# NEUROINFORMATICS-GROUP-FAV-KIV-ZCU/EEG_DataAnalysisPackage

Measured on AMD Instinct MI355X. Metric: epochs/sec feature-extracted (whole node) + % HBM roofline, 1/2/4/8 GPUs, higher is better.
Workload: dtype f64

## Files before the change

### eeg_dataanalysispackage_amd/csrc/nn.hip

```cpp
#include <hip/hip_runtime.h>

#include <algorithm>
#include <cstdint>

#include "eegfx.h"
#include "launch.h"

namespace eegfx {

constexpr int kNnThreads = 256;
constexpr int kNnMaxTileRows = 64;
constexpr int kNnMinStagedRows = 8;
constexpr int kNnLdsBytes = 147456;
constexpr int kNnGridCap = 768;
constexpr int kNnAccRegs = 4;
constexpr int kNnPartialDoubles = 8388608;
constexpr int kNnValidateThreads = 256;
constexpr int kNnValidateMaxBlocks = 4096;
constexpr int kNnStatThreads = 256;
constexpr int kNnStatUnroll = 4;
constexpr int kNnStatMaxBlocks = 2048;
constexpr int kNnDirThreads = 1024;

namespace dev {

__device__ __forceinline__ double nn_act(int act, double z) {
  switch (act) {
    case EEGFX_NN_ACT_TANH: return tanh(z);
    case EEGFX_NN_ACT_RELU: return z > 0.0 ? z : (z == z ? 0.0 : z);
    case EEGFX_NN_ACT_IDENTITY: return z;
    case EEGFX_NN_ACT_SOFTPLUS: return (z > 0.0 ? z : 0.0) + log1p(exp(-fabs(z)));
    case EEGFX_NN_ACT_ELU: return z > 0.0 ? z : expm1(z);
    default: return 1.0 / (1.0 + exp(-z));
  }
}

__device__ __forceinline__ double nn_dact(int act, double z, double a) {
  switch (act) {
    case EEGFX_NN_ACT_TANH: return 1.0 - a * a;
    case EEGFX_NN_ACT_RELU: return z > 0.0 ? 1.0 : 0.0;
    case EEGFX_NN_ACT_IDENTITY: return 1.0;
    case EEGFX_NN_ACT_SOFTPLUS: return 1.0 / (1.0 + exp(-z));
    case EEGFX_NN_ACT_ELU: return z > 0.0 ? 1.0 : exp(z);
    default: return a * (1.0 - a);
  }
}

__device__ __forceinline__ double nn_dot(const double* a, const double* w, int ws, int n,
                                         double z) {
  for (int i = 0; i < n; ++i) z = __builtin_fma(a[i], w[(int64_t)i * ws], z);
  return z;
}

__device__ __forceinline__ void nn_stage_weights(const NnNet& net, const NnTile& tl, double* lds,
                                                 const double* __restrict__ params) {
  const int t = threadIdx.x;
  for (int l = 0; l < net.L; ++l) {
    const int no = net.n_out[l], nw = net.n_in[l] * no;
    const double* src = params + net.w_off[l];
    if (l > 0 || tl.w1_lds) {
      int i = t / no, j = t - i * no;
      const int di = kNnThreads / no, dj = kNnThreads - di * no;
      for (int e = t; e < nw; e += kNnThreads) {
        lds[tl.w_lds[l] + i * tl.w_stride[l] + j] = src[e];
        i += di;
        j += dj;
        if (j >= no) {
          j -= no;
          ++i;
        }
      }
    }
    for (int j = t; j < no; j += kNnThreads) lds[tl.b_lds[l] + j] = src[nw + j];
  }
}

__device__ __forceinline__ void nn_load_rows(const NnNet& net, const NnTile& tl, double* lds,
                                             const double* __restrict__ X,
                                             const double* __restrict__ y, int64_t row0,
                                             int rows) {
  const int t = threadIdx.x, d = net.d;
  const double* src = X + row0 * d;
  int r = t / d, c = t - r * d;
  const int dr = kNnThreads / d, dc = kNnThreads - dr * d;
  for (int e = t; e < rows * d; e += kNnThreads) {
    lds[tl.x_off + r * tl.x_stride + c] = src[e];
    r += dr;
    c += dc;
    if (c >= d) {
      c -= d;
      ++r;
    }
  }
  if (y && t < rows) lds[tl.y_off + t] = y[row0 + t];
}

__device__ __forceinline__ void nn_forward(const NnNet& net, const NnTile& tl, double* lds,
                                           const double* __restrict__ params, int rows) {
  const int t = threadIdx.x;
  for (int l = 0; l < net.L; ++l) {
    const int no = net.n_out[l], ni = net.n_in[l], act = net.act[l];
    const int in_off = l == 0 ? tl.x_off : tl.a_off[l - 1];
    const int in_stride = l == 0 ? tl.x_stride : tl.a_stride[l - 1];
    const int os = tl.a_stride[l];
    int r = t / no, j = t - r * no;
    const int dr = kNnThreads / no, dj = kNnThreads - dr * no;
    for (int e = t; e < rows * no; e += kNnThreads) {
      const double* a = lds + in_off + r * in_stride;
      double z = lds[tl.b_lds[l] + j];
      if (l == 0 && !tl.w1_lds)
        z = nn_dot(a, params + net.w_off[0] + j, no, ni, z);
      else
        z = nn_dot(a, lds + tl.w_lds[l] + j, tl.w_stride[l], ni, z);
      lds[tl.z_off[l] + r * os + j] = z;
      if (act != EEGFX_NN_ACT_SOFTMAX) lds[tl.a_off[l] + r * os + j] = nn_act(act, z);
      r += dr;
      j += dj;
      if (j >= no) {
        j -= no;
        ++r;
      }
    }
    __syncthreads();
    if (act == EEGFX_NN_ACT_SOFTMAX) {
      if (t < rows) {
        const double* z = lds + tl.z_off[l] + t * os;
        double* a = lds + tl.a_off[l] + t * os;
        double m = z[0];
        for (int j2 = 1; j2 < no; ++j2) m = fmax(m, z[j2]);
        double s = 0.0;
        for (int j2 = 0; j2 < no; ++j2) {
          const double ez = exp(z[j2] - m);
          a[j2] = ez;
          s += ez;
        }
        for (int j2 = 0; j2 < no; ++j2) a[j2] = a[j2] / s;
      }
      __syncthreads();
    }
  }
}

struct NnTerm {
  int a_off, a_stride, d_off, d_stride;
};
__device__ __forceinline__ NnTerm nn_term(const NnNet& net, const NnTile& tl, int p) {
  int l = 0;
  for (int k = 1; k < net.L; ++k)
    if (p >= net.w_off[k]) l = k;
  const int q = p - net.w_off[l], no = net.n_out[l], nw = net.n_in[l] * no;
  NnTerm tm;
  tm.d_stride = tl.a_stride[l];
  if (q < nw) {
    const int i = q / no;
    tm.d_off = tl.z_off[l] + (q - i * no);
    tm.a_off = (l == 0 ? tl.x_off : tl.a_off[l - 1]) + i;
    tm.a_stride = l == 0 ? tl.x_stride : tl.a_stride[l - 1];
  } else {
    tm.d_off = tl.z_off[l] + (q - nw);
    tm.a_off = -1;
    tm.a_stride = 0;
  }
  return tm;
}
__device__ __forceinline__ double nn_term_sum(const double* lds, const NnTerm& tm, int rows,
                                              double acc) {
  if (tm.a_off >= 0) {
    for (int r = 0; r < rows; ++r)
      acc = __builtin_fma(lds[tm.a_off + r * tm.a_stride], lds[tm.d_off + r * tm.d_stride], acc);
  } else {
    for (int r = 0; r < rows; ++r) acc += lds[tm.d_off + r * tm.d_stride];
  }
  return acc;
}

__device__ __forceinline__ double nn_row_loss(int kind, double p0, double p1, double y0, double y1,
                                              double* g0, double* g1) {
  switch (kind) {
    case EEGFX_NN_LOSS_XENT:
      *g0 = -y0 / p0 + (1.0 - y0) / (1.0 - p0);
      *g1 = -y1 / p1 + (1.0 - y1) / (1.0 - p1);
      return -((y0 * log(p0) + (1.0 - y0) * log(1.0 - p0)) +
               (y1 * log(p1) + (1.0 - y1) * log(1.0 - p1)));
    case EEGFX_NN_LOSS_NLL:
      *g0 = -y0 / p0;
      *g1 = -y1 / p1;
      return -(y0 * log(p0) + y1 * log(p1));
    case EEGFX_NN_LOSS_SQUARED:
      *g0 = 2.0 * (p0 - y0);
      *g1 = 2.0 * (p1 - y1);
      return (p0 - y0) * (p0 - y0) + (p1 - y1) * (p1 - y1);
    default:
      *g0 = p0 - y0;
      *g1 = p1 - y1;
      return ((p0 - y0) * (p0 - y0) + (p1 - y1) * (p1 - y1)) / 2.0;
  }
}

__device__ __forceinline__ void nn_store_loss(const NnTile& tl, double* lds, double my_loss,
                                              double* out) {
  const int t = threadIdx.x;
  __syncthreads();
  if (t < kNnMaxTileRows) lds[tl.loss_off + t] = my_loss;
  __syncthreads();
  if (t == 0) {
    double s = 0.0;
    for (int r = 0; r < kNnMaxTileRows; ++r) s += lds[tl.loss_off + r];
    *out = s;
  }
}

__global__ __launch_bounds__(kNnThreads) void nn_grad_kernel(
    const double* __restrict__ X, const double* __restrict__ y, int64_t n, const NnNet net,
    const NnTile tl, const NnState* __restrict__ st, double* __restrict__ partial) {
  if (st->flag) return;
  extern __shared__ __attribute__((aligned(16))) double nn_lds[];
  double* lds = nn_lds;
  const double* params = (const double*)(st + 1);
  const int t = threadIdx.x, P = net.P, L = net.L;
  double* slab = partial + (int64_t)blockIdx.x * (P + 1);
  nn_stage_weights(net, tl, lds, params);
  NnTerm term[kNnAccRegs];
  double acc[kNnAccRegs];
#pragma unroll
  for (int k = 0; k < kNnAccRegs; ++k) {
    acc[k] = 0.0;
    const int p = t + k * kNnThreads;
    term[k] = nn_term(net, tl, p < P ? p : 0);
  }
  for (int p = t + kNnAccRegs * kNnThreads; p < P; p += kNnThreads) slab[p] = 0.0;
  double my_loss = 0.0;
  const int last = L - 1, out_act = net.act[last];
  for (int64_t row0 = (int64_t)blockIdx.x * tl.rows; row0 < n;
       row0 += (int64_t)gridDim.x * tl.rows) {
    const int rows = (int)(n - row0 < tl.rows ? n - row0 : tl.rows);
    __syncthreads();
    nn_load_rows(net, tl, lds, X, y, row0, rows);
    __syncthreads();
    nn_forward(net, tl, lds, params, rows);
    if (t < rows) {
      const int os = tl.a_stride[last];
      double* z = lds + tl.z_off[last] + t * os;
      const double p0 = lds[tl.a_off[last] + t * os], p1 = lds[tl.a_off[last] + t * os + 1];
      const double y0 = lds[tl.y_off + t], y1 = fabs(1.0 - y0);
      double g0, g1;
      const double loss = nn_row_loss(net.loss, p0, p1, y0, y1, &g0, &g1);
      my_loss += loss;
      double d0, d1;
      if ((net.loss == EEGFX_NN_LOSS_XENT && out_act == EEGFX_NN_ACT_SIGMOID) ||
          (net.loss == EEGFX_NN_LOSS_NLL && out_act == EEGFX_NN_ACT_SOFTMAX)) {
        d0 = p0 - y0;
        d1 = p1 - y1;
      } else if (out_act == EEGFX_NN_ACT_SOFTMAX) {
        const double gp = g0 * p0 + g1 * p1;
        d0 = p0 * (g0 - gp);
        d1 = p1 * (g1 - gp);
      } else {
        d0 = g0 * nn_dact(out_act, z[0], p0);
        d1 = g1 * nn_dact(out_act, z[1], p1);
      }
      z[0] = d0;
      z[1] = d1;
    }
    __syncthreads();
    for (int l = last; l >= 1; --l) {
      const int ni = net.n_in[l], no = net.n_out[l], act = net.act[l - 1];
      const int ps = tl.a_stride[l - 1];
      int r = t / ni, i = t - r * ni;
      const int dr = kNnThreads / ni, di = kNnThreads - dr * ni;
      for (int e = t; e < rows * ni; e += kNnThreads) {
        const double s = nn_dot(lds + tl.z_off[l] + r * tl.a_stride[l],
                                lds + tl.w_lds[l] + i * tl.w_stride[l], 1, no, 0.0);
        double* zp = lds + tl.z_off[l - 1] + r * ps + i;
        *zp = act == EEGFX_NN_ACT_SOFTMAX
                  ? s
                  : s * nn_dact(act, *zp, lds[tl.a_off[l - 1] + r * ps + i]);
        r += dr;
        i += di;
        if (i >= ni) {
          i -= ni;
          ++r;
        }
      }
      __syncthreads();
      if (act == EEGFX_NN_ACT_SOFTMAX) {
        if (t < rows) {
          double* s = lds + tl.z_off[l - 1] + t * ps;
          const double* a = lds + tl.a_off[l - 1] + t * ps;
          double sa = 0.0;
          for (int m = 0; m < ni; ++m) sa = __builtin_fma(s[m], a[m], sa);
          for (int m = 0; m < ni; ++m) s[m] = a[m] * (s[m] - sa);
        }
        __syncthreads();
      }
    }
#pragma unroll
    for (int k = 0; k < kNnAccRegs; ++k)
      if (t + k * kNnThreads < P) acc[k] = nn_term_sum(lds, term[k], rows, acc[k]);
    for (int p = t + kNnAccRegs * kNnThreads; p < P; p += kNnThreads)
      slab[p] = nn_term_sum(lds, nn_term(net, tl, p), rows, slab[p]);
  }
#pragma unroll
  for (int k = 0; k < kNnAccRegs; ++k)
    if (t + k * kNnThreads < P) slab[t + k * kNnThreads] = acc[k];
  nn_store_loss(tl, lds, my_loss, slab + P);
}

__device__ __forceinline__ double nn_updater(int updater, double lr, double mu, int it, double g,
                                             double* s1, double* s2) {
  switch (updater) {
    case EEGFX_NN_UPD_SGD:
      return lr * g;
    case EEGFX_NN_UPD_ADAM: {
      const double b1 = 0.9, b2 = 0.999, t = (double)(it + 1);
      const double m = b1 * *s1 + (1.0 - b1) * g;
      const double v = b2 * *s2 + (1.0 - b2) * (g * g);
      *s1 = m;
      *s2 = v;
      return lr * sqrt(1.0 - pow(b2, t)) / (1.0 - pow(b1, t)) * (m / (sqrt(v) + 1e-8));
    }
    case EEGFX_NN_UPD_ADAGRAD: {
      const double h = *s1 + g * g;
      *s1 = h;
      return lr * g / (sqrt(h) + 1e-6);
    }
    case EEGFX_NN_UPD_RMSPROP: {
      const double r = 0.95 * *s1 + 0.05 * (g * g);
      *s1 = r;
      return lr * g / sqrt(r + 1e-8);
    }
    default: {
      const double v = *s1, vn = mu * v - lr * g;
      *s1 = vn;
      return mu * v - (1.0 + mu) * vn;
    }
  }
}

enum { kVecG = 0, kVecGNew = 1, kVecDir = 2, kVecCand = 3, kVecPOld = 4, kVecGOld = 5,
       kVecS = 6, kVecY = kVecS + kNnLbfgsM };
__device__ __forceinline__ double* nn_opt_vec(const NnOpt* opt, int k, int P) {
  return (double*)(opt + 1) + (int64_t)k * P;
}

__device__ __forceinline__ double nn_partial_mean(const double* __restrict__ partial, int G,
                                                  int64_t n, int P, int p) {
  const int64_t stride = P + 1;
  double s = 0.0;
  for (int b = 0; b < G; ++b) s += partial[b * stride + p];
  return s / (double)n;
}

__device__ __forceinline__ bool nn_last_workgroup(uint32_t* ticket) {
  __syncthreads();
  if (threadIdx.x != 0) return false;
  __threadfence();
  if (atomicAdd(ticket, 1u) != gridDim.x - 1) return false;
  *ticket = 0;
  return true;
}

template <bool OPT>
__global__ __launch_bounds__(kNnThreads) void nn_update_kernel(
    const double* __restrict__ partial, int G, int64_t n, int P, int updater, double lr,
    double mu, NnState* __restrict__ st, NnOpt* __restrict__ opt, double* __restrict__ scores) {
  if (st->flag) return;
  const int it = st->iter;
  const int p = blockIdx.x * kNnThreads + threadIdx.x;
  if (p < P) {
    const double g = nn_partial_mean(partial, G, n, P, p);
    double* w = (double*)(st + 1) + p;
    double* s1 = w + P;
    double* s2 = s1 + P;
    const double u = nn_updater(updater, lr, mu, it, g, s1, s2);
    if constexpr (OPT)
      nn_opt_vec(opt, kVecGNew, P)[p] = u;
    else
      *w = *w - u;
  }
  if (blockIdx.x == 0 && threadIdx.x == 0) {
    if constexpr (OPT)
      opt->score_new = nn_partial_mean(partial, G, n, P, P);
    else if (scores)
      scores[it] = nn_partial_mean(partial, G, n, P, P);
  }
  if (nn_last_workgroup(&st->ticket)) st->iter = it + 1;
}

__device__ __forceinline__ double nn_move(double p, double step, double d) { return p - step * d; }
__device__ __forceinline__ bool nn_finite(double v) { return fabs(v) <= 1.7976931348623157e308; }

__global__ __launch_bounds__(kNnThreads) void nn_score_kernel(
    const double* __restrict__ X, const double* __restrict__ y, int64_t n, const NnNet net,
    const NnTile tl, const NnState* __restrict__ st, const NnOpt* __restrict__ opt,
    double* __restrict__ partial) {
  if (st->flag || opt->line.done) return;
  extern __shared__ __attribute__((aligned(16))) double nn_lds[];
  double* lds = nn_lds;
  const double* params = nn_opt_vec(opt, kVecCand, net.P);
  const int t = threadIdx.x, last = net.L - 1;
  nn_stage_weights(net, tl, lds, params);
  double my_loss = 0.0;
  for (int64_t row0 = (int64_t)blockIdx.x * tl.rows; row0 < n;
       row0 += (int64_t)gridDim.x * tl.rows) {
    const int rows = (int)(n - row0 < tl.rows ? n - row0 : tl.rows);
    __syncthreads();
    nn_load_rows(net, tl, lds, X, y, row0, rows);
    __syncthreads();
    nn_forward(net, tl, lds, params, rows);
    if (t < rows) {
      const int os = tl.a_stride[last];
      const double p0 = lds[tl.a_off[last] + t * os], p1 = lds[tl.a_off[last] + t * os + 1];
      const double y0 = lds[tl.y_off + t], y1 = fabs(1.0 - y0);
      double g0, g1;
      my_loss += nn_row_loss(net.loss, p0, p1, y0, y1, &g0, &g1);
    }
  }
  nn_store_loss(tl, lds, my_loss, partial + (int64_t)blockIdx.x * (net.P + 1) + net.P);
}

__device__ __forceinline__ int nn_line_step(NnLine& ln, double sc, int max_ls, double* move,
                                            NnSearchRec* rec) {
  const double s0 = ln.s0, slope = ln.slope, step = ln.step, prev = ln.sc;
  ln.sc = sc;
  ln.trials += 1;
  rec->trials = ln.trials;
  rec->pad = 0;
  if (sc < ln.best) {
    ln.best = sc;
    ln.best_step = step;
  }
  if (sc <= s0 + 1e-4 * step * slope) {
    ln.done = 1;
    rec->step = *move = step;
    rec->score = sc;
    return 1;
  }
  double tmp;
  if (!nn_finite(sc) || !nn_finite(prev)) {
    tmp = 0.2 * step;
  } else if (step == 1.0) {
    tmp = -slope / (2.0 * (sc - s0 - slope));
  } else {
    const double step2 = ln.step2;
    const double r1 = sc - s0 - step * slope, r2 = ln.sc2 - s0 - step2 * slope;
    const double q1 = r1 / (step * step), q2 = r2 / (step2 * step2);
    const double a = (q1 - q2) / (step - step2);
    const double b = (-step2 * q1 + step * q2) / (step - step2);
    if (a == 0.0) {
      tmp = -slope / (2.0 * b);
    } else {
      const double disc = b * b - 3.0 * a * slope;
      if (disc < 0.0)
        tmp = 0.5 * step;
      else if (b <= 0.0)
        tmp = (-b + sqrt(disc)) / (3.0 * a);
      else
        tmp = -slope / (b + sqrt(disc));
    }
    if (!(tmp < 0.5 * step)) tmp = 0.5 * step;
  }
  ln.step2 = step;
  ln.sc2 = sc;
  ln.step = tmp > 0.1 * step ? tmp : 0.1 * step;
  if (ln.trials < max_ls && !(ln.step < ln.step_min)) {
    *move = ln.step;
    return 0;
  }
  ln.done = 1;
  if (ln.trials == max_ls && ln.best < s0) {
    rec->step = *move = ln.best_step;
    rec->score = ln.best;
    return 1;
  }
  rec->step = *move = 0.0;
  rec->score = s0;
  return 2;
}

__global__ __launch_bounds__(kNnThreads) void nn_search_kernel(
    const double* __restrict__ partial, int G, int64_t n, int P, int max_ls,
    NnState* __restrict__ st, NnOpt* __restrict__ opt, NnSearchRec* __restrict__ search) {
  if (st->flag || opt->line.done) return;
  __shared__ double sh_move;
  __shared__ int sh_mode;
  NnLine ln;
  NnSearchRec rec;
  int it = 0;
  if (threadIdx.x == 0) {
    ln = opt->line;
    it = opt->it;
    double move;
    sh_mode = nn_line_step(ln, nn_partial_mean(partial, G, n, P, P), max_ls, &move, &rec);
    sh_move = move;
  }
  __syncthreads();
  const int mode = sh_mode, k = blockIdx.x * kNnThreads + threadIdx.x;
  if (k < P && mode != 2) {
    double* p = (double*)(st + 1);
    const double v = nn_move(p[k], sh_move, nn_opt_vec(opt, kVecDir, P)[k]);
    if (mode == 1)
      p[k] = v;
    else
      nn_opt_vec(opt, kVecCand, P)[k] = v;
  }
  if (nn_last_workgroup(&opt->ticket)) {
    opt->line = ln;
    if (ln.done) search[it] = rec;
  }
}

template <int N>
__device__ __forceinline__ void nn_block_sum(double (&v)[N], double* red) {
  const int t = threadIdx.x;
#pragma unroll
  for (int k = 0; k < N; ++k) red[k * kNnDirThreads + t] = v[k];
  __syncthreads();
  for (int h = kNnDirThreads / 2; h > 0; h >>= 1) {
    if (t < h) {
#pragma unroll
      for (int k = 0; k < N; ++k) red[k * kNnDirThreads + t] += red[k * kNnDirThreads + t + h];
    }
    __syncthreads();
  }
#pragma unroll
  for (int k = 0; k < N; ++k) v[k] = red[k * kNnDirThreads];
  __syncthreads();
}
__device__ __forceinline__ double nn_block_max(double v, double* red) {
  const int t = threadIdx.x;
  red[t] = v;
  __syncthreads();
  for (int h = kNnDirThreads / 2; h > 0; h >>= 1) {
    if (t < h && (red[t + h] > red[t] || red[t + h] != red[t + h])) red[t] = red[t + h];
    __syncthreads();
  }
  v = red[0];
  __syncthreads();
  return v;
}

__global__ __launch_bounds__(kNnDirThreads) void nn_direction_kernel(
    int P, int algo, int iters, int first, NnState* __restrict__ st, NnOpt* __restrict__ opt,
    double* __restrict__ scores, NnSearchRec* __restrict__ search) {
  if (st->flag) return;
  __shared__ double red[3 * kNnDirThreads];
  constexpr int D = kNnDirThreads, M = kNnLbfgsM;
  const int t = threadIdx.x;
  const double* p = (const double*)(st + 1);
  double* g = nn_opt_vec(opt, kVecG, P);
  const double* gn = nn_opt_vec(opt, kVecGNew, P);
  double* dir = nn_opt_vec(opt, kVecDir, P);
  double* p_old = nn_opt_vec(opt, kVecPOld, P);
  double* g_old = nn_opt_vec(opt, kVecGOld, P);
  const int it = first ? -1 : opt->it;
  const double old = opt->score, score = opt->score_new;
  int hist = opt->hist, head = opt->head;
  double rho_new = 0.0;
  bool stop = false;
  const bool lbfgs = algo == EEGFX_NN_OPT_LBFGS;
  if (first) {
    for (int k = t; k < P; k += D) {
      const double v = gn[k];
      g[k] = v;
      dir[k] = v;
      if (lbfgs) {
        p_old[k] = p[k];
        g_old[k] = v;
      }
    }
  } else {
    if (algo == EEGFX_NN_OPT_CG) {
      double v[2] = {0.0, 0.0};
      for (int k = t; k < P; k += D) {
        v[0] += (gn[k] - g[k]) * gn[k];
        v[1] += g[k] * g[k];
      }
      nn_block_sum(v, red);
      const double q = v[0] / v[1], gamma = q < 0.0 ? 0.0 : q;
      for (int k = t; k < P; k += D) dir[k] = gamma * dir[k] + gn[k];
    } else if (lbfgs) {
      head = hist == 0 ? 0 : (head + 1) % M;
      hist = hist < M ? hist + 1 : M;
      double* s_new = nn_opt_vec(opt, kVecS + head, P);
      double* y_new = nn_opt_vec(opt, kVecY + head, P);
      double v[2] = {0.0, 0.0};
      for (int k = t; k < P; k += D) {
        const double s = p[k] - p_old[k], yv = gn[k] - g_old[k];
        s_new[k] = s;
        y_new[k] = yv;
        v[0] += s * yv;
        v[1] += yv * yv;
        dir[k] = gn[k];
        p_old[k] = p[k];
        g_old[k] = gn[k];
      }
      nn_block_sum(v, red);
      const double sy = v[0] + 1e-5, yy = v[1] + 1e-5;
      rho_new = 1.0 / sy;
      double a[M];
#pragma unroll
      for (int j = 0; j < M; ++j) {
        a[j] = 0.0;
        if (j < hist) {
          const int slot = (head - j + M) % M;
          const double* sv = nn_opt_vec(opt, kVecS + slot, P);
          const double* yv = nn_opt_vec(opt, kVecY + slot, P);
          double d[1] = {0.0};
          for (int k = t; k < P; k += D) d[0] += sv[k] * dir[k];
          nn_block_sum(d, red);
          a[j] = (j == 0 ? rho_new : opt->rho[slot]) * d[0];
          for (int k = t; k < P; k += D) dir[k] -= a[j] * yv[k];
        }
      }
      const double scale = sy / yy;
      for (int k = t; k < P; k += D) dir[k] *= scale;
#pragma unroll
      for (int j = M - 1; j >= 0; --j) {
        if (j < hist) {
          const int slot = (head - j + M) % M;
          const double* sv = nn_opt_vec(opt, kVecS + slot, P);
          const double* yv = nn_opt_vec(opt, kVecY + slot, P);
          double d[1] = {0.0};
          for (int k = t; k < P; k += D) d[0] += yv[k] * dir[k];
          nn_block_sum(d, red);
          const double b = (j == 0 ? rho_new : opt->rho[slot]) * d[0];
          for (int k = t; k < P; k += D) dir[k] += (a[j] - b) * sv[k];
        }
      }
    } else {
      for (int k = t; k < P; k += D) dir[k] = gn[k];
    }
    double asum[1] = {0.0};
    for (int k = t; k < P; k += D) {
      const double v = gn[k];
      g[k] = v;
      asum[0] += fabs(v);
    }
    nn_block_sum(asum, red);
    stop = asum[0] == 0.0;
    if (!(score == 0.0 && old == 0.0) &&
        2.0 * fabs(old - score) <= 1e-5 * (fabs(old) + fabs(score) + 1e-4))
      stop = true;
  }
  const int next = it + 1;
  const bool search_next = !stop && next < iters;
  NnLine ln{};
  if (search_next) {
    double v[2] = {0.0, 0.0};
    double test = 0.0;
    for (int k = t; k < P; k += D) {
      v[0] += dir[k] * dir[k];
      v[1] += dir[k] * g[k];
      const double ap = fabs(p[k]), q = fabs(g[k]) / (ap > 1.0 ? ap : 1.0);
      if (q > test || q != q) test = q;
    }
    nn_block_sum(v, red);
    test = nn_block_max(test, red);
    const double norm = sqrt(v[0]);
    if (norm > 100.0) {
      const double f = 100.0 / norm;
      for (int k = t; k < P; k += D) dir[k] *= f;
    }
    ln.s0 = ln.sc = ln.sc2 = ln.best = score;
    ln.slope = -v[1];
    ln.step_min = 1e-7 / test;
    ln.step = ln.best_step = 1.0;
    ln.step2 = 0.0;
    ln.done = ln.step < ln.step_min ? 1 : 0;
    if (!ln.done) {
      double* cand = nn_opt_vec(opt, kVecCand, P);
      for (int k = t; k < P; k += D) cand[k] = nn_move(p[k], 1.0, dir[k]);
    }
  }
  __syncthreads();
  if (t == 0) {
    opt->score = score;
    if (!first) {
      opt->iterations_run = next;
      if (lbfgs) {
        opt->hist = hist;
        opt->head = head;
        opt->rho[head] = rho_new;
      }
    }
    if (stop) st->flag = 1;
    if (search_next) {
      opt->it = next;
      opt->line = ln;
      if (scores) scores[next] = score;
      if (ln.done) search[next] = NnSearchRec{0.0, score, 0, 0};
    }
  }
}

__global__ __launch_bounds__(kNnThreads) void nn_predict_kernel(
    const double* __restrict__ X, int64_t n, const NnNet net, const NnTile tl,
    const double* __restrict__ params, double* __restrict__ out) {
  extern __shared__ __attribute__((aligned(16))) double nn_lds[];
  double* lds = nn_lds;
  const int t = threadIdx.x, last = net.L - 1;
  nn_stage_weights(net, tl, lds, params);
  for (int64_t row0 = (int64_t)blockIdx.x * tl.rows; row0 < n;
       row0 += (int64_t)gridDim.x * tl.rows) {
    const int rows = (int)(n - row0 < tl.rows ? n - row0 : tl.rows);
    __syncthreads();
    nn_load_rows(net, tl, lds, X, nullptr, row0, rows);
    __syncthreads();
    nn_forward(net, tl, lds, params, rows);
    if (t < rows) out[row0 + t] = lds[tl.a_off[last] + t * tl.a_stride[last]];
  }
}

__global__ __launch_bounds__(kNnValidateThreads) void nn_validate_kernel(
    const double* __restrict__ y, int64_t n, NnState* __restrict__ st) {
  for (int64_t i = (int64_t)blockIdx.x * blockDim.x + threadIdx.x; i < n;
       i += (int64_t)gridDim.x * blockDim.x)
    if (!(y[i] == 0.0 || y[i] == 1.0)) st->flag = 2;
}

__device__ __forceinline__ long long java_round(double x) {
  if (x != x) return 0;
  if (x >= 9223372036854775807.0) return 0x7FFFFFFFFFFFFFFFLL;
  if (x <= -9223372036854775808.0) return -0x7FFFFFFFFFFFFFFFLL - 1;
  const double f = floor(x);
  return (long long)f + (x - f >= 0.5 ? 1 : 0);
}

__device__ __forceinline__ unsigned long long nn_wave_sum(unsigned long long v) {
#pragma unroll
  for (int off = 32; off > 0; off >>= 1) v += __shfl_down(v, off, 64);
  return v;
}

__global__ __launch_bounds__(kNnStatThreads) void nn_stats_kernel(
    const double* __restrict__ scores, const double* __restrict__ labels, int64_t n,
    NnStatsOut* __restrict__ out, double* __restrict__ sums) {
  constexpr int U = kNnStatUnroll;
  __shared__ double red[3][kNnStatThreads];
  unsigned long long cell[4] = {0, 0, 0, 0};
  double acc[3] = {0.0, 0.0, 0.0};
  const int64_t step = (int64_t)gridDim.x * blockDim.x;
  for (int64_t r = (int64_t)blockIdx.x * blockDim.x + threadIdx.x; r < n; r += step * U) {
    double a[U], s[U];
#pragma unroll
    for (int u = 0; u < U; ++u) {
      const bool live = r + u * step < n;
      a[u] = live ? labels[r + u * step] : 0.0;
      s[u] = live ? scores[r + u * step] : 0.0;
    }
#pragma unroll
    for (int u = 0; u < U; ++u) {
      if (r + u * step >= n) continue;
      acc[0] += (a[u] - s[u]) * (a[u] - s[u]);
      const long long want = java_round(a[u]), got = java_round(s[u]);
      if (want == 0) {
        cell[got == 0 ? 1 : 2] += 1;
        acc[1] += s[u];
      } else if (want == 1) {
        cell[got == 1 ? 0 : 3] += 1;
        acc[2] += s[u];
      }
    }
  }
#pragma unroll
  for (int k = 0; k < 4; ++k) {
    const unsigned long long s = nn_wave_sum(cell[k]);
    if ((threadIdx.x & 63) == 0 && s) atomicAdd(&out->cell[k], s);
  }
#pragma unroll
  for (int k = 0; k < 3; ++k) red[k][threadIdx.x] = acc[k];
  __syncthreads();
  for (int h = kNnStatThreads / 2; h > 0; h >>= 1) {
    if ((int)threadIdx.x < h) {
#pragma unroll
      for (int k = 0; k < 3; ++k) red[k][threadIdx.x] += red[k][threadIdx.x + h];
    }
    __syncthreads();
  }
  if (threadIdx.x < 3) sums[blockIdx.x * 3 + threadIdx.x] = red[threadIdx.x][0];
}

}

NnTile nn_plan_tile(const NnNet& net) {
  auto odd = [](int v) { return v | 1; };
  NnTile t{};
  t.x_stride = odd(net.d);
  int per_row = t.x_stride + 2;
  int fixed = kNnMaxTileRows;
  for (int l = 0; l < net.L; ++l) {
    t.w_stride[l] = odd(net.n_out[l]);
    t.a_stride[l] = odd(net.n_out[l]);
    per_row += 2 * t.a_stride[l];
    fixed += net.n_out[l];
    if (l > 0) fixed += net.n_in[l] * t.w_stride[l];
  }
  const int budget = kNnLdsBytes / (int)sizeof(double);
  const int w1 = net.n_in[0] * t.w_stride[0];
  const int with_w1 = (budget - fixed - w1) / per_row;
  t.w1_lds = with_w1 >= kNnMinStagedRows ? 1 : 0;
  if (t.w1_lds) fixed += w1;
  t.rows = std::min(kNnMaxTileRows, (budget - fixed) / per_row);
  int off = 0;
  auto take = [&](int doubles) {
    const int at = off;
    off += doubles;
    return at;
  };
  t.loss_off = take(kNnMaxTileRows);
  for (int l = 0; l < net.L; ++l) {
    t.w_lds[l] = (l > 0 || t.w1_lds) ? take(net.n_in[l] * t.w_stride[l]) : 0;
    t.b_lds[l] = take(net.n_out[l]);
  }
  t.y_off = take(t.rows);
  t.x_off = take(t.rows * t.x_stride);
  for (int l = 0; l < net.L; ++l) {
    t.a_off[l] = take(t.rows * t.a_stride[l]);
    t.z_off[l] = take(t.rows * t.a_stride[l]);
  }
  t.doubles = off;
  return t;
}

int nn_grid(int64_t n, const NnNet& net, const NnTile& tl) {
  const int64_t tiles = (n + tl.rows - 1) / tl.rows;
  const int64_t cap = std::min<int64_t>(kNnGridCap, std::max(1, kNnPartialDoubles / (net.P + 1)));
  return (int)std::max<int64_t>(1, std::min(tiles, cap));
}

template <typename K>
static hipError_t nn_allow_lds(K kernel) {
  return hipFuncSetAttribute((const void*)kernel, hipFuncAttributeMaxDynamicSharedMemorySize,
                             kNnLdsBytes);
}

hipError_t launch_nn_validate(hipStream_t st, const double* y, int64_t n, NnState* state) {
  hipLaunchKernelGGL(dev::nn_validate_kernel,
                     dim3(grid_for(n, kNnValidateThreads, kNnValidateMaxBlocks)),
                     dim3(kNnValidateThreads), 0, st, y, n, state);
  return hipGetLastError();
}

static dim3 nn_param_grid(int P) { return dim3((P + kNnThreads - 1) / kNnThreads); }

hipError_t launch_nn_gradient(hipStream_t st, const double* X, const double* y, int64_t n,
                              const NnNet& net, const NnTile& tl, int G, NnState* state,
                              double* partial, double lr, double momentum, NnOpt* opt,
                              double* scores) {
  hipError_t e = nn_allow_lds(dev::nn_grad_kernel);
  if (e != hipSuccess) return e;
  hipLaunchKernelGGL(dev::nn_grad_kernel, dim3(G), dim3(kNnThreads),
                     sizeof(double) * (size_t)tl.doubles, st, X, y, n, net, tl, state, partial);
  e = hipGetLastError();
  if (e != hipSuccess) return e;
  hipLaunchKernelGGL(opt ? dev::nn_update_kernel<true> : dev::nn_update_kernel<false>,
                     nn_param_grid(net.P), dim3(kNnThreads), 0, st, partial, G, n, net.P,
                     net.updater, lr, momentum, state, opt, scores);
  return hipGetLastError();
}

hipError_t launch_nn_trial(hipStream_t st, const double* X, const double* y, int64_t n,
                           const NnNet& net, const NnTile& tl, int G, NnState* state, NnOpt* opt,
                           double* partial, int max_ls, NnSearchRec* search) {
  hipError_t e = nn_allow_lds(dev::nn_score_kernel);
  if (e != hipSuccess) return e;
  hipLaunchKernelGGL(dev::nn_score_kernel, dim3(G), dim3(kNnThreads),
                     sizeof(double) * (size_t)tl.doubles, st, X, y, n, net, tl, state, opt,
                     partial);
  e = hipGetLastError();
  if (e != hipSuccess) return e;
  hipLaunchKernelGGL(dev::nn_search_kernel, nn_param_grid(net.P), dim3(kNnThreads), 0, st,
                     partial, G, n, net.P, max_ls, state, opt, search);
  return hipGetLastError();
}

hipError_t launch_nn_direction(hipStream_t st, const NnNet& net, int algorithm, int iterations,
                               bool first, NnState* state, NnOpt* opt, double* scores,
                               NnSearchRec* search) {
  hipLaunchKernelGGL(dev::nn_direction_kernel, dim3(1), dim3(kNnDirThreads), 0, st, net.P,
                     algorithm, iterations, first ? 1 : 0, state, opt, scores, search);
  return hipGetLastError();
}

hipError_t launch_nn_predict(hipStream_t st, const double* X, int64_t n, const NnNet& net,
                             const NnTile& tl, const double* params, double* out) {
  if (n == 0) return hipSuccess;
  hipError_t e = nn_allow_lds(dev::nn_predict_kernel);
  if (e != hipSuccess) return e;
  const int64_t tiles = (n + tl.rows - 1) / tl.rows;
  hipLaunchKernelGGL(dev::nn_predict_kernel, dim3((unsigned)std::min<int64_t>(tiles, kNnGridCap)),
                     dim3(kNnThreads), sizeof(double) * (size_t)tl.doubles, st, X, n, net, tl,
                     params, out);
  return hipGetLastError();
}

int nn_stats_grid(int64_t n) {
  return (int)grid_for(n, kNnStatThreads * kNnStatUnroll, kNnStatMaxBlocks);
}

hipError_t launch_nn_stats(hipStream_t st, const double* scores, const double* labels, int64_t n,
                           NnStatsOut* out, double* sums) {
  if (n == 0) return hipSuccess;
  hipLaunchKernelGGL(dev::nn_stats_kernel, dim3(nn_stats_grid(n)), dim3(kNnStatThreads), 0, st,
                     scores, labels, n, out, sums);
  return hipGetLastError();
}

}
```

Measured before the change: 1.153 billion.

## Use f64 MFMA fragments for forward, backprop and weight-gradient accumulation

Replaces the per-element scalar FMA dot products in the forward pass, the backward delta propagation and the weight-gradient reduction with 16x16x4 f64 MFMA fragments, spread across waves. Weight-gradient accumulators are now held per wave as MFMA fragments, bias gradients get a dedicated per-thread reduction, and row loading is batched to keep more global loads in flight. Launch bounds now request higher occupancy. The cost is that small layer widths get padded into 16-wide fragments, and the larger accumulator arrays raise register pressure.

```diff
diff --git a/eeg_dataanalysispackage_amd/csrc/nn.hip b/eeg_dataanalysispackage_amd/csrc/nn.hip
--- a/eeg_dataanalysispackage_amd/csrc/nn.hip
+++ b/eeg_dataanalysispackage_amd/csrc/nn.hip
@@ -13,7 +13,7 @@
 constexpr int kNnMinStagedRows = 8;
 constexpr int kNnLdsBytes = 147456;
 constexpr int kNnGridCap = 768;
-constexpr int kNnAccRegs = 4;
+constexpr int kNnAccRegs = 16;
 constexpr int kNnPartialDoubles = 8388608;
 constexpr int kNnValidateThreads = 256;
 constexpr int kNnValidateMaxBlocks = 4096;
@@ -21,6 +21,11 @@
 constexpr int kNnStatUnroll = 4;
 constexpr int kNnStatMaxBlocks = 2048;
 constexpr int kNnDirThreads = 1024;
+constexpr int kNnWaves = kNnThreads / 64;
+constexpr int kNnLoadAhead = 12;
+constexpr int kNnStepsAhead = 2;
+constexpr int kNnFrag = 16;
+constexpr int kNnAccFrags = kNnAccRegs / 4;
 
 namespace dev {
 
@@ -46,11 +51,56 @@
   }
 }
 
-__device__ __forceinline__ double nn_dot(const double* a, const double* w, int ws, int n,
-                                         double z) {
-  for (int i = 0; i < n; ++i) z = __builtin_fma(a[i], w[(int64_t)i * ws], z);
-  return z;
-}
+typedef double NnAcc __attribute__((ext_vector_type(4)));
+
+__device__ __forceinline__ int nn_frags(int n) { return (n + kNnFrag - 1) / kNnFrag; }
+__device__ __forceinline__ int nn_wave() {
+  return __builtin_amdgcn_readfirstlane((int)threadIdx.x >> 6);
+}
+
+__device__ __forceinline__ NnAcc nn_mma(const double* a, int a_ms, int a_ks, int M,
+                                        const double* b, int b_ks, int b_ns, int N, int K,
+                                        NnAcc c) {
+  const int lane = threadIdx.x & 63, q = lane >> 4, x = lane & 15;
+  const bool a_in = x < M, b_in = x < N;
+  const int a_at = x * a_ms, b_at = x * b_ns;
+  for (int k0 = 0; k0 < K; k0 += 4 * kNnStepsAhead) {
+    double av[kNnStepsAhead], bv[kNnStepsAhead];
+#pragma unroll
+    for (int u = 0; u < kNnStepsAhead; ++u) {
+      const int k = k0 + 4 * u + q;
+      const bool a_ok = a_in && k < K, b_ok = b_in && k < K;
+      av[u] = a[a_ok ? a_at + k * a_ks : 0];
+      bv[u] = b[b_ok ? b_at + k * b_ks : 0];
+      av[u] = a_ok ? av[u] : 0.0;
+      bv[u] = b_ok ? bv[u] : 0.0;
+    }
+#pragma unroll
+    for (int u = 0; u < kNnStepsAhead; ++u)
+      if (k0 + 4 * u < K) c = __builtin_amdgcn_mfma_f64_16x16x4f64(av[u], bv[u], c, 0, 0, 0);
+  }
+  return c;
+}
+
+struct NnFragWalk {
+  int m0, n0, left;
+  __device__ __forceinline__ NnFragWalk(int M, int N)
+      : m0(0), n0(nn_wave() * kNnFrag), left(nn_frags(M)) {
+    wrap(nn_frags(N) * kNnFrag);
+  }
+  __device__ __forceinline__ void wrap(int width) {
+    while (n0 >= width && left > 0) {
+      n0 -= width;
+      m0 += kNnFrag;
+      --left;
+    }
+  }
+  __device__ __forceinline__ bool more() const { return left > 0; }
+  __device__ __forceinline__ void next(int N) {
+    n0 += kNnWaves * kNnFrag;
+    wrap(nn_frags(N) * kNnFrag);
+  }
+};
 
 __device__ __forceinline__ void nn_stage_weights(const NnNet& net, const NnTile& tl, double* lds,
                                                  const double* __restrict__ params) {
@@ -81,15 +131,25 @@
                                              int rows) {
   const int t = threadIdx.x, d = net.d;
   const double* src = X + row0 * d;
+  const int total = rows * d;
   int r = t / d, c = t - r * d;
   const int dr = kNnThreads / d, dc = kNnThreads - dr * d;
-  for (int e = t; e < rows * d; e += kNnThreads) {
-    lds[tl.x_off + r * tl.x_stride + c] = src[e];
-    r += dr;
-    c += dc;
-    if (c >= d) {
-      c -= d;
-      ++r;
+  for (int e0 = t; e0 < total; e0 += kNnLoadAhead * kNnThreads) {
+    double v[kNnLoadAhead];
+#pragma unroll
+    for (int u = 0; u < kNnLoadAhead; ++u) {
+      const int e = e0 + u * kNnThreads;
+      v[u] = e < total ? src[e] : 0.0;
+    }
+#pragma unroll
+    for (int u = 0; u < kNnLoadAhead; ++u) {
+      if (e0 + u * kNnThreads < total) lds[tl.x_off + r * tl.x_stride + c] = v[u];
+      r += dr;
+      c += dc;
+      if (c >= d) {
+        c -= d;
+        ++r;
+      }
     }
   }
   if (y && t < rows) lds[tl.y_off + t] = y[row0 + t];
@@ -103,22 +163,27 @@
     const int in_off = l == 0 ? tl.x_off : tl.a_off[l - 1];
     const int in_stride = l == 0 ? tl.x_stride : tl.a_stride[l - 1];
     const int os = tl.a_stride[l];
-    int r = t / no, j = t - r * no;
-    const int dr = kNnThreads / no, dj = kNnThreads - dr * no;
-    for (int e = t; e < rows * no; e += kNnThreads) {
-      const double* a = lds + in_off + r * in_stride;
-      double z = lds[tl.b_lds[l] + j];
+    const int q = (t & 63) >> 4, col_in = t & 15;
+    for (NnFragWalk f(rows, no); f.more(); f.next(no)) {
+      const int col = f.n0 + col_in;
+      const bool live = col < no;
+      const double bias = lds[tl.b_lds[l] + (live ? col : 0)];
+      NnAcc z;
+      z[0] = z[1] = z[2] = z[3] = live ? bias : 0.0;
+      const double* a = lds + in_off + f.m0 * in_stride;
       if (l == 0 && !tl.w1_lds)
-        z = nn_dot(a, params + net.w_off[0] + j, no, ni, z);
+        z = nn_mma(a, in_stride, 1, rows - f.m0, params + net.w_off[0] + f.n0, no, 1, no - f.n0,
+                   ni, z);
       else
-        z = nn_dot(a, lds + tl.w_lds[l] + j, tl.w_stride[l], ni, z);
-      lds[tl.z_off[l] + r * os + j] = z;
-      if (act != EEGFX_NN_ACT_SOFTMAX) lds[tl.a_off[l] + r * os + j] = nn_act(act, z);
-      r += dr;
-      j += dj;
-      if (j >= no) {
-        j -= no;
-        ++r;
+        z = nn_mma(a, in_stride, 1, rows - f.m0, lds + tl.w_lds[l] + f.n0, tl.w_stride[l], 1,
+                   no - f.n0, ni, z);
+#pragma unroll
+      for (int k = 0; k < 4; ++k) {
+        const int r = f.m0 + q + 4 * k;
+        if (r < rows && live) {
+          lds[tl.z_off[l] + r * os + col] = z[k];
+          if (act != EEGFX_NN_ACT_SOFTMAX) lds[tl.a_off[l] + r * os + col] = nn_act(act, z[k]);
+        }
       }
     }
     __syncthreads();
@@ -141,37 +206,44 @@
   }
 }
 
-struct NnTerm {
-  int a_off, a_stride, d_off, d_stride;
+struct NnGradFrag {
+  int l, m0, n0;
 };
-__device__ __forceinline__ NnTerm nn_term(const NnNet& net, const NnTile& tl, int p) {
-  int l = 0;
-  for (int k = 1; k < net.L; ++k)
-    if (p >= net.w_off[k]) l = k;
-  const int q = p - net.w_off[l], no = net.n_out[l], nw = net.n_in[l] * no;
-  NnTerm tm;
-  tm.d_stride = tl.a_stride[l];
-  if (q < nw) {
-    const int i = q / no;
-    tm.d_off = tl.z_off[l] + (q - i * no);
-    tm.a_off = (l == 0 ? tl.x_off : tl.a_off[l - 1]) + i;
-    tm.a_stride = l == 0 ? tl.x_stride : tl.a_stride[l - 1];
-  } else {
-    tm.d_off = tl.z_off[l] + (q - nw);
-    tm.a_off = -1;
-    tm.a_stride = 0;
-  }
-  return tm;
-}
-__device__ __forceinline__ double nn_term_sum(const double* lds, const NnTerm& tm, int rows,
-                                              double acc) {
-  if (tm.a_off >= 0) {
-    for (int r = 0; r < rows; ++r)
-      acc = __builtin_fma(lds[tm.a_off + r * tm.a_stride], lds[tm.d_off + r * tm.d_stride], acc);
-  } else {
-    for (int r = 0; r < rows; ++r) acc += lds[tm.d_off + r * tm.d_stride];
-  }
-  return acc;
+__device__ __forceinline__ NnGradFrag nn_grad_frag(const NnNet& net, int g) {
+  for (int l = 0; l < net.L; ++l) {
+    const int across = nn_frags(net.n_out[l]), count = nn_frags(net.n_in[l]) * across;
+    if (g < count) return NnGradFrag{l, g / across * kNnFrag, g % across * kNnFrag};
+    g -= count;
+  }
+  return NnGradFrag{-1, 0, 0};
+}
+__device__ __forceinline__ NnAcc nn_grad_mma(const NnNet& net, const NnTile& tl, const double* lds,
+                                             const NnGradFrag& f, int rows, NnAcc acc) {
+  const int l = f.l;
+  const int a_off = l == 0 ? tl.x_off : tl.a_off[l - 1];
+  const int a_stride = l == 0 ? tl.x_stride : tl.a_stride[l - 1];
+  return nn_mma(lds + a_off + f.m0, 1, a_stride, net.n_in[l] - f.m0, lds + tl.z_off[l] + f.n0,
+                tl.a_stride[l], 1, net.n_out[l] - f.n0, rows, acc);
+}
+__device__ __forceinline__ NnAcc nn_frag_load(const NnNet& net, const NnGradFrag& f,
+                                              const double* grad) {
+  const int lane = threadIdx.x & 63, j = f.n0 + (lane & 15), no = net.n_out[f.l];
+  NnAcc c;
+#pragma unroll
+  for (int k = 0; k < 4; ++k) {
+    const int i = f.m0 + (lane >> 4) + 4 * k;
+    c[k] = i < net.n_in[f.l] && j < no ? grad[net.w_off[f.l] + i * no + j] : 0.0;
+  }
+  return c;
+}
+__device__ __forceinline__ void nn_frag_store(const NnNet& net, const NnGradFrag& f, double* grad,
+                                              NnAcc c) {
+  const int lane = threadIdx.x & 63, j = f.n0 + (lane & 15), no = net.n_out[f.l];
+#pragma unroll
+  for (int k = 0; k < 4; ++k) {
+    const int i = f.m0 + (lane >> 4) + 4 * k;
+    if (i < net.n_in[f.l] && j < no) grad[net.w_off[f.l] + i * no + j] = c[k];
+  }
 }
 
 __device__ __forceinline__ double nn_row_loss(int kind, double p0, double p1, double y0, double y1,
@@ -210,7 +282,7 @@
   }
 }
 
-__global__ __launch_bounds__(kNnThreads) void nn_grad_kernel(
+__global__ __launch_bounds__(kNnThreads, 3) void nn_grad_kernel(
     const double* __restrict__ X, const double* __restrict__ y, int64_t n, const NnNet net,
     const NnTile tl, const NnState* __restrict__ st, double* __restrict__ partial) {
   if (st->flag) return;
@@ -220,15 +292,29 @@
   const int t = threadIdx.x, P = net.P, L = net.L;
   double* slab = partial + (int64_t)blockIdx.x * (P + 1);
   nn_stage_weights(net, tl, lds, params);
-  NnTerm term[kNnAccRegs];
-  double acc[kNnAccRegs];
-#pragma unroll
-  for (int k = 0; k < kNnAccRegs; ++k) {
-    acc[k] = 0.0;
-    const int p = t + k * kNnThreads;
-    term[k] = nn_term(net, tl, p < P ? p : 0);
-  }
-  for (int p = t + kNnAccRegs * kNnThreads; p < P; p += kNnThreads) slab[p] = 0.0;
+  const int wave = nn_wave();
+  NnGradFrag frag[kNnAccFrags];
+  NnAcc acc[kNnAccFrags];
+  const NnAcc zero = {0.0, 0.0, 0.0, 0.0};
+#pragma unroll
+  for (int k = 0; k < kNnAccFrags; ++k) {
+    frag[k] = nn_grad_frag(net, wave + k * kNnWaves);
+    acc[k] = zero;
+  }
+  for (int g = wave + kNnAccFrags * kNnWaves;; g += kNnWaves) {
+    const NnGradFrag f = nn_grad_frag(net, g);
+    if (f.l < 0) break;
+    nn_frag_store(net, f, slab, zero);
+  }
+  static_assert(kNnMaxLayers * kNnMaxWidth <= kNnThreads, "a thread for every bias");
+  int bias_at = -1, bias_stride = 0, bias_p = 0;
+  for (int l = 0, first = 0; l < L; first += net.n_out[l], ++l)
+    if (t >= first && t < first + net.n_out[l]) {
+      bias_at = tl.z_off[l] + t - first;
+      bias_stride = tl.a_stride[l];
+      bias_p = net.w_off[l] + net.n_in[l] * net.n_out[l] + t - first;
+    }
+  double bias_acc = 0.0;
   double my_loss = 0.0;
   const int last = L - 1, out_act = net.act[last];
   for (int64_t row0 = (int64_t)blockIdx.x * tl.rows; row0 < n;
@@ -266,20 +352,22 @@
     for (int l = last; l >= 1; --l) {
       const int ni = net.n_in[l], no = net.n_out[l], act = net.act[l - 1];
       const int ps = tl.a_stride[l - 1];
-      int r = t / ni, i = t - r * ni;
-      const int dr = kNnThreads / ni, di = kNnThreads - dr * ni;
-      for (int e = t; e < rows * ni; e += kNnThreads) {
-        const double s = nn_dot(lds + tl.z_off[l] + r * tl.a_stride[l],
-                                lds + tl.w_lds[l] + i * tl.w_stride[l], 1, no, 0.0);
-        double* zp = lds + tl.z_off[l - 1] + r * ps + i;
-        *zp = act == EEGFX_NN_ACT_SOFTMAX
-                  ? s
-                  : s * nn_dact(act, *zp, lds[tl.a_off[l - 1] + r * ps + i]);
-        r += dr;
-        i += di;
-        if (i >= ni) {
-          i -= ni;
-          ++r;
+      const int q = (t & 63) >> 4, col_in = t & 15;
+      for (NnFragWalk f(rows, ni); f.more(); f.next(ni)) {
+        NnAcc s;
+        s[0] = s[1] = s[2] = s[3] = 0.0;
+        s = nn_mma(lds + tl.z_off[l] + f.m0 * tl.a_stride[l], tl.a_stride[l], 1, rows - f.m0,
+                   lds + tl.w_lds[l] + f.n0 * tl.w_stride[l], 1, tl.w_stride[l], ni - f.n0, no, s);
+        const int i = f.n0 + col_in;
+#pragma unroll
+        for (int k = 0; k < 4; ++k) {
+          const int r = f.m0 + q + 4 * k;
+          if (r < rows && i < ni) {
+            double* zp = lds + tl.z_off[l - 1] + r * ps + i;
+            *zp = act == EEGFX_NN_ACT_SOFTMAX
+                      ? s[k]
+                      : s[k] * nn_dact(act, *zp, lds[tl.a_off[l - 1] + r * ps + i]);
+          }
         }
       }
       __syncthreads();
@@ -294,15 +382,23 @@
         __syncthreads();
       }
     }
-#pragma unroll
-    for (int k = 0; k < kNnAccRegs; ++k)
-      if (t + k * kNnThreads < P) acc[k] = nn_term_sum(lds, term[k], rows, acc[k]);
-    for (int p = t + kNnAccRegs * kNnThreads; p < P; p += kNnThreads)
-      slab[p] = nn_term_sum(lds, nn_term(net, tl, p), rows, slab[p]);
-  }
-#pragma unroll
-  for (int k = 0; k < kNnAccRegs; ++k)
-    if (t + k * kNnThreads < P) slab[t + k * kNnThreads] = acc[k];
+    if (bias_at >= 0) {
+#pragma unroll 8
+      for (int r = 0; r < rows; ++r) bias_acc += lds[bias_at + r * bias_stride];
+    }
+#pragma unroll
+    for (int k = 0; k < kNnAccFrags; ++k)
+      if (frag[k].l >= 0) acc[k] = nn_grad_mma(net, tl, lds, frag[k], rows, acc[k]);
+    for (int g = wave + kNnAccFrags * kNnWaves;; g += kNnWaves) {
+      const NnGradFrag f = nn_grad_frag(net, g);
+      if (f.l < 0) break;
+      nn_frag_store(net, f, slab, nn_grad_mma(net, tl, lds, f, rows, nn_frag_load(net, f, slab)));
+    }
+  }
+#pragma unroll
+  for (int k = 0; k < kNnAccFrags; ++k)
+    if (frag[k].l >= 0) nn_frag_store(net, frag[k], slab, acc[k]);
+  if (bias_at >= 0) slab[bias_p] = bias_acc;
   nn_store_loss(tl, lds, my_loss, slab + P);
 }
 
```

Result: no change. 1.153 billion, median of 4 (+0.1%).
